# mit-acl/dpgo_ros

Measured on AMD Instinct MI355X. Metric: ms/RBCD-iteration + iterations-to-1e-6-relcost, sphere2500 5-agent, lower is better.
Workload: dtype f64; 1 GPU; sphere2500.g2o, 5 agents, synchronous round-robin RBCD, RGD(step 0.2, dense preconditioner) + Nesterov (restart 20), r=5, library weighting; mid-run iterations one launch each (k_step_fd: the private part of an agent's preconditioner product formed by the launch before its own, its row products by the one before that), hipGraphs of up to 256 iterations; agents=5, poses_per_agent=500, placement=agent a on rank a % N

## Files before the change

### dpgo_ros_amd/csrc/kernels.h

```cpp
#pragma once
#include <hip/hip_runtime.h>
#include "dpgo_dev.h"

namespace dpgo {

struct LaunchCtx {
  int r;
  hipStream_t stream;
  const AgentDev *agents;
  TeamDev *team;
  int ny = 1;
  int dense_max_n = 1 << 30;
  bool any_two_level = false;
  int tl_max_wg = 0;
  const int *host_precond = nullptr;
  const AgentDev *host_agents = nullptr;
  int num_agents = 0;
  bool bake_desc = false;
  const int *up_slots = nullptr;
  const double *up_in = nullptr;
  int up_n0 = 0, up_n1 = 0;
  int max_lds = 160 * 1024;
  int stage_cap = 0;
  const NestState *nest_all = nullptr;
// ... 29 lines not shown
void launch_eval_report(const LaunchCtx &c, int sel, int max_n, int xb, int egb, int gfb, int poff, const EvalOpts &o,
                        const ReportTail &rt);
size_t eval_staged_lds_bytes(int r, int cap);
constexpr int EVS_STATIC_LDS = 8 * 1024;
void launch_hess(const LaunchCtx &c, int sel, int max_n, int xb, int egb, int vb, int ob, int poff);
void launch_precond(const LaunchCtx &c, int sel, int max_n, int mode, int xb, int vb, int zb, int sp, int max_inner,
                    double step, int accel, int num_robots, int advance = PADV_NONE, int restart_interval = 1, int ahead = 0);
void launch_eval_stats(const LaunchCtx &c, int max_n, int first, int has_eval, int has_stats, int num_robots,
                       int restart_interval, int eval_sel = SEL_SCHED, int stats_sel = SEL_SCHED, const NestState *nest_copy = nullptr);
bool step_fe_supported(int r);
int step_fe_max_edges();
void launch_step_fe(const LaunchCtx &c, int sel, int next_sel, double step, int num_robots, int restart_interval,
                    const NestState *nest_src, NestState *nest_dst, int parity, int next2_sel = -1, int carry = 0);
int step_fe_carry_max_poses();
int step_fd_pick_m0(int min_private_chunks);
void launch_fd_open(const LaunchCtx &c, int m0, int s0, int s1, double *pacc_out);
void launch_fd_prime(const LaunchCtx &c, int s0, int s1, int s2, int max_n, int num_robots, int restart_interval, const NestState *nest_src);
void launch_step_fd(const LaunchCtx &c, int m0, int sel, int next_sel, int next2_sel, int next3_sel, double step, int num_robots,
                    int restart_interval, const NestState *nest_src, NestState *nest_dst, int parity, int flags,
                    const double *pacc_in, double *pacc_out);
constexpr int LS_MAX_TRIALS = 8;
void launch_ls_trials(const LaunchCtx &c, int sel, int max_n, int dirb, double step0, double shrink, int ntrials);
void launch_ls_cost(const LaunchCtx &c, int sel, int max_n, int dirb, int ntrials);
void launch_ls_apply(const LaunchCtx &c, int sel, int max_n, double step0, double shrink, double sigma, int ntrials, int tail = 0,
                     int num_robots = 1, int restart_interval = 1);
void launch_tcg_hv(const LaunchCtx &c, int sel, int max_n, int sp, int max_inner);
void launch_retract(const LaunchCtx &c, int sel, int max_n, int xb, int eb, double scale, int ob, int guard_state);
void launch_project_raw(const LaunchCtx &c, const double *X, double *out, int n);
void launch_tangent_raw(const LaunchCtx &c, const double *X, const double *V, double *out, int n);
void launch_retract_raw(const LaunchCtx &c, const double *X, const double *E, double *out, int n);
// ... 70 lines not shown
```

### dpgo_ros_amd/csrc/step_deep.hip

```cpp
#include "kernel_common.h"
#include <algorithm>

namespace dpgo {

constexpr int FD_KC = 2048;
#ifndef DPGO_FD_HEAD
#define DPGO_FD_HEAD 0
#endif
#ifndef DPGO_FD_GC_LATE
#define DPGO_FD_GC_LATE 0
#endif
#ifndef DPGO_FD_PACC_WT
#define DPGO_FD_PACC_WT 0
#endif
#ifndef DPGO_FD_E_EARLY
#define DPGO_FD_E_EARLY 0
#endif
#ifndef DPGO_FD_KA_PREFETCH
#define DPGO_FD_KA_PREFETCH 1
#endif
constexpr int FD_HEAD = DPGO_FD_HEAD;

enum { FD_SY_C = 0, FD_SY_E, FD_SY_D, FD_SY_F, FD_SY_N, FD_SY_RQ, FD_SY_COUNT = 8 };

__device__ __forceinline__ void fd_signal(int *cnt) {
  __builtin_amdgcn_fence(__ATOMIC_RELEASE, "workgroup", "local");
  if ((threadIdx.x & 63) == 0) __hip_atomic_fetch_add(cnt, 1, __ATOMIC_RELAXED, __HIP_MEMORY_SCOPE_WORKGROUP);
}

__device__ __forceinline__ void fd_signal_requested(int *cnt) {
  __builtin_amdgcn_sched_barrier(0);
  asm volatile("" ::: "memory");
  if ((threadIdx.x & 63) == 0) __hip_atomic_fetch_add(cnt, 1, __ATOMIC_RELAXED, __HIP_MEMORY_SCOPE_WORKGROUP);
  asm volatile("" ::: "memory");
  __builtin_amdgcn_sched_barrier(0);
}
// ... 8 lines not shown
__device__ __forceinline__ int fd_pos_off(const unsigned char *ord, int pose) {
  const int ch = pose >> 4;
  int p = 0;
#pragma unroll
  for (int i = 0; i < 32; ++i) p = ((int)ord[i] == ch) ? i : p;
  return p * 64 * R + (pose & 15) * 4 * R;
}

template <int R>
struct FdXn {
  double2 v[3][2 * R];
};

template <int R>
__device__ __forceinline__ void fd_xn_request(const AgentDev &ag, const FeBases &fb, int parity, int ln, FdXn<R> &xr) {
#pragma unroll
  for (int q = 0; q < 3; ++q) {
    {
      unsigned wsel = 0;
#pragma unroll
      for (int k = 0; k < 32; ++k) {
        const unsigned wk = ag.fe_code[(32 * q + k < FE_MAX_EDGES / 2) ? 32 * q + k : FE_MAX_EDGES / 2 - 1];
        wsel = ((ln >> 1) == k) ? wk : wsel;
      }
      const unsigned code = (ln & 1) ? (wsel >> 16) : (wsel & 0xffffu);
      const int sa = (int)(code >> 12), sf = (int)(code & 0xfffu);
      const double *yb = fb.ybase[0];
      int yn = fb.npose[0];
#pragma unroll
      for (int k = 1; k < LOOKAHEAD_MAX_AGENTS; ++k) { yb = (sa == k) ? fb.ybase[k] : yb; yn = (sa == k) ? fb.npose[k] : yn; }
      const double *xp = yb + (parity ? (size_t)B_ALT * 4 * R * yn : (size_t)0) + (size_t)sf * 4 * R;
#pragma unroll
      for (int k = 0; k < 2 * R; ++k) xr.v[q][k] = ld2(xp + 2 * k);
    }
  }
}

template <int R>
__device__ __forceinline__ void fd_xn_to_lds(const AgentDev &ag, int ln, const FdXn<R> &xr, double *Es) {
  constexpr int EPE = 4 * R + 16;
  int nsh = ag.nshared;
  asm volatile("" : "+v"(nsh));
#pragma unroll
  for (int q = 0; q < 3; ++q) {
    if (64 * q < nsh && 64 * q + ln < nsh) {
      double *E = Es + (size_t)(64 * q + ln) * EPE;
#pragma unroll
      for (int k = 0; k < 2 * R; ++k) *reinterpret_cast<double2 *>(E + 2 * k) = xr.v[q][k];
    }
  }
}

struct FdCf {
  static constexpr int TRIPS = FE_MAX_EDGES * 8 / 64;
  double2 v[TRIPS];
};

__device__ __forceinline__ void fd_cf_request(const AgentDev &ag, int ln, FdCf &cr) {
  const int nit = ag.nshared * 8;
#pragma unroll
  for (int j = 0; j < FdCf::TRIPS; ++j) cr.v[j] = ld2(ag.fe_coef + 2 * min(64 * j + ln, nit - 1));
}

template <int R>
__device__ __forceinline__ void fd_cf_to_lds(const AgentDev &ag, int ln, const FdCf &cr, double *Es) {
  constexpr int EPE = 4 * R + 16;
  int nit = ag.nshared * 8;
  asm volatile("" : "+v"(nit));
#pragma unroll
  for (int j = 0; j < FdCf::TRIPS; ++j) {
    const int t = 64 * j + ln;
    if (64 * j < nit && t < nit) *reinterpret_cast<double2 *>(Es + (size_t)(t >> 3) * EPE + 4 * R + 2 * (t & 7)) = cr.v[j];
  }
}

template <int R, int NC>
struct FdCur {
  double2 mc[NC];
  double pa[R];
};

template <int R, int M0, int NC>
__device__ __forceinline__ void fd_cur_request(const AgentDev &ag, const double *pacc_in, int bx, int nblk, int l, FdCur<R, NC> &cu) {
  const int cg = (l >> 5) & 7, kl = l & 31;
  const int N4 = ag.N4, col = 8 * bx + cg;
  const double *Mc = ag.M + (size_t)((col < N4) ? col : 0) * N4;
#pragma unroll
  for (int i = 0; i < NC; ++i) cu.mc[i] = ld2_nt(Mc + min(2 * kl + 64 * (int)ag.fe_ord[M0 + i], N4 - 2));
#pragma unroll
  for (int a = 0; a < R; ++a) cu.pa[a] = gp(pacc_in)[((size_t)min(bx, nblk - 1) * R + a) * 256 + l];
}

template <int R, int M0, int NC>
__device__ __forceinline__ void fd_cur_product(const FdCur<R, NC> &cu, const double *vs, double *red, int l) {
  const int cg = (l >> 5) & 7, kl = l & 31;
  double acc[R];
#pragma unroll
  for (int a = 0; a < R; ++a) acc[a] = cu.pa[a];
#pragma unroll
  for (int i = 0; i < NC; ++i) {
    const int k = 2 * kl + 64 * (M0 + i);
    double wv[2 * R];
#pragma unroll
    for (int q = 0; q < R; ++q) {
      const double2 t2 = *reinterpret_cast<const double2 *>(&vs[k * R + 2 * q]);
      wv[2 * q] = t2.x; wv[2 * q + 1] = t2.y;
    }
#pragma unroll
    for (int a = 0; a < R; ++a) acc[a] = __builtin_fma(wv[R + a], cu.mc[i].y, __builtin_fma(wv[a], cu.mc[i].x, acc[a]));
  }
#pragma unroll
  for (int a = 0; a < R; ++a) red[kl * (8 * R + 1) + cg * R + a] = acc[a];
}

#ifdef DPGO_FE_TRACE
#ifndef DPGO_FE_TRACE_BLOCK
#define DPGO_FE_TRACE_BLOCK 100
#endif
#define FD_TRACE_DECL __shared__ unsigned long long fd_stamps[8 * 16];
#ifndef DPGO_FD_STAMP_MASK
#define DPGO_FD_STAMP_MASK 0xFFFF
#endif
#define FD_STAMP(k) do { if (((DPGO_FD_STAMP_MASK >> (k)) & 1) && (threadIdx.x & 63) == 0) fd_stamps[(threadIdx.x >> 6) * 16 + (k)] = wall_clock64(); } while (0)
#define FD_FLUSH() do { if ((threadIdx.x & 63) == 0) { const int w_ = threadIdx.x >> 6; \
    if (blockIdx.x == DPGO_FE_TRACE_BLOCK) for (int k_ = 0; k_ < 16; ++k_) ag.part[PART_E + 4000 * PART_STRIDE + w_ * 16 + k_] = (double)fd_stamps[w_ * 16 + k_]; \
    if (w_ == 4) { ag.part[PART_E + (4100 + 2 * (int)blockIdx.x) * PART_STRIDE] = (double)fd_stamps[4 * 16]; ag.part[PART_E + (4100 + 2 * (int)blockIdx.x) * PART_STRIDE + 1] = (double)fd_stamps[4 * 16 + 15]; } \
    if (w_ == 0) { ag.part[PART_E + (4100 + 2 * (int)blockIdx.x) * PART_STRIDE + 2] = (double)fd_stamps[15]; } } } while (0)
#elif defined(DPGO_FD_ENDS)
#define FD_TRACE_DECL
#define FD_STAMP(k) do { if ((k) == 0 && blockIdx.x == 100 && threadIdx.x == 256) ag.part[PART_E + 4000 * PART_STRIDE + 64] = (double)wall_clock64(); } while (0)
#define FD_FLUSH() do { if (blockIdx.x == 100 && (threadIdx.x & 63) == 0) ag.part[PART_E + 4000 * PART_STRIDE + (threadIdx.x >> 6) * 16 + 15] = (double)wall_clock64(); } while (0)
#else
#define FD_TRACE_DECL
#define FD_STAMP(k) do { } while (0)
#define FD_FLUSH() do { } while (0)
#endif

template <int R, int M0>
__global__ __launch_bounds__(512) void k_step_fd(TeamDev *team, int sel, int next_sel, double step, int num_robots, int restart_interval,
                                                 const NestState *nest_src, NestState *nest_dst, int parity, const AgentDev agv,
                                                 int next3_sel, int flags, const FdNext nx, const FeBases fb,
                                                 const double *__restrict__ pacc_in, double *__restrict__ pacc_out, int nblk_all,
                                                 int num_agents) {
  const AgentDev &ag = agv;
#if DPGO_FD_KA_PREFETCH
  {
    const unsigned *ka = (const unsigned *)__builtin_amdgcn_kernarg_segment_ptr();
    constexpr int KA_LINES = (int)((sizeof(AgentDev) + sizeof(FdNext) + sizeof(FeBases) + 160 + 63) / 64);
    unsigned touch = 0;
#pragma unroll
    for (int i = 0; i < KA_LINES; ++i) touch |= ka[16 * i];
    asm volatile("" ::"s"(touch));
  }
#endif
  const double *__restrict__ Xr = ag.buf[parity ? B_XALT : B_X];
  const double *__restrict__ Yr = ag.buf[parity ? B_YALT : B_Y];
  double *__restrict__ Xw = ag.buf[parity ? B_X : B_XALT];
  double *__restrict__ Yw = ag.buf[parity ? B_Y : B_YALT];
  const int hb = (int)blockIdx.x;
  const int bx = (hb % 8) * ((int)gridDim.x / 8) + hb / 8;
  const int tid = threadIdx.x;
  const int N4 = ag.N4, n = ag.n;
  const int nblk = (N4 + 7) / 8;
  if (bx >= nblk_all) return;
  const bool own = bx < nblk, in = (flags & FD_IN) != 0;
  constexpr int KC = FD_KC, MREG = KC / 64, NC = MREG - M0;
  __shared__ double vs[R * KC];
  __shared__ double zs[8 * R];
  __shared__ double red[32 * (8 * R + 1)];
  __shared__ double Ysh[2 * 4 * R];
  __shared__ double Esh[2][2 * 4 * R];
  __shared__ double Es[FE_MAX_EDGES * (4 * R + 16)];
  __shared__ double tl_x[2 * 4 * R], tl_v[2 * 4 * R], tl_y[2 * 4 * R], tl_s[2 * 16];
  __shared__ double Ex[2 * 3 * 4 * R];
  __shared__ double Psh[2 * 4 * R], tl_rel[2];
  __shared__ int sy[FD_SY_COUNT];
  FD_TRACE_DECL
  FD_STAMP(0);
  if (tid < FD_SY_COUNT) sy[tid] = 0;
  lds_barrier();
  const int pj0 = own ? 2 * bx : 0, pj1 = (own && 2 * bx + 1 < n) ? 2 * bx + 1 : -1;
  const int npose = own ? ((pj1 >= 0) ? 2 : 1) : 0;
  constexpr int EPE = 4 * R + 16;
  const int cwv = __builtin_amdgcn_readfirstlane(tid >> 6), ln = tid & 63;

  if (cwv < 4) {
    const int cg = (tid >> 5) & 7, kl = tid & 31;
    for (int t = N4 * R + tid; t < KC * R; t += 256) vs[t] = 0.0;
    constexpr int NGC = ((KC - 64 * M0) * R / 2 + 255) / 256;
    double2 gc[NGC];
#if !DPGO_FD_GC_LATE
    {
      const double *Gc = ag.buf[B_CARRY_G];
#pragma unroll
      for (int u = 0; u < NGC; ++u) gc[u] = ld2(Gc + min(M0 * 64 * R + 2 * (tid + 256 * u), N4 * R - 2));
    }
#endif
    const int cold = 8 * bx + cg;
    const int N4d = nx.N4d;
    const double *Md = nx.Md + (size_t)((cold < N4d) ? cold : 0) * N4d;
    double2 mn[M0];
#pragma unroll
    for (int i = 0; i < FD_HEAD; ++i) mn[i] = ld2_nt(Md + min(2 * kl + 64 * (int)nx.ord_d[i], N4d - 2));
    FD_STAMP(10);
    __builtin_amdgcn_sched_barrier(0);
#if DPGO_FD_GC_LATE
    {
      const double *Gc = ag.buf[B_CARRY_G];
#pragma unroll
      for (int u = 0; u < NGC; ++u) gc[u] = ld2(Gc + min(M0 * 64 * R + 2 * (tid + 256 * u), N4 * R - 2));
    }
#endif
#pragma unroll
    for (int u = 0; u < NGC; ++u) {
      const int tt = M0 * 64 * R + 2 * (tid + 256 * u);
      if (tt < N4 * R) *reinterpret_cast<double2 *>(&vs[tt]) = gc[u];
    }
    fd_signal(&sy[FD_SY_C]);
    FD_STAMP(1);
    fd_wait(&sy[FD_SY_RQ], 4);
    FD_STAMP(11);
    __builtin_amdgcn_sched_barrier(0);
    asm volatile("" ::: "memory");
    constexpr int NGN = (M0 * 64 * R / 2 + 255) / 256;
    double2 gn[NGN];
#pragma unroll
    for (int u = 0; u < NGN; ++u) gn[u] = ld2(nx.Gd + min(2 * (tid + 256 * u), M0 * 64 * R - 2));
#pragma unroll
    for (int i = FD_HEAD; i < M0; ++i) mn[i] = ld2_nt(Md + min(2 * kl + 64 * (int)nx.ord_d[i], N4d - 2));
    FD_STAMP(12);
#pragma unroll
    for (int u = 0; u < NGN; ++u) {
      const int tt = 2 * (tid + 256 * u);
      if (tt < M0 * 64 * R) *reinterpret_cast<double2 *>(&vs[tt]) = gn[u];
    }
    fd_signal(&sy[FD_SY_N]);
    fd_wait(&sy[FD_SY_N], 4);
    fd_wait(&sy[FD_SY_F], 4);
    FD_STAMP(13);
    double acc[R];
#pragma unroll
    for (int a = 0; a < R; ++a) acc[a] = 0;
#pragma unroll
    for (int i = 0; i < M0; ++i) {
      const int k = 2 * kl + 64 * i;
      double wv[2 * R];
#pragma unroll
      for (int q = 0; q < R; ++q) {
        const double2 t2 = *reinterpret_cast<const double2 *>(&vs[k * R + 2 * q]);
        wv[2 * q] = t2.x; wv[2 * q + 1] = t2.y;
      }
#pragma unroll
      for (int a = 0; a < R; ++a) acc[a] = __builtin_fma(wv[R + a], mn[i].y, __builtin_fma(wv[a], mn[i].x, acc[a]));
    }
    if ((flags & FD_P) && bx < nx.nblk_d) {
#pragma unroll
#if DPGO_FD_PACC_WT
      for (int a = 0; a < R; ++a) st_c(pacc_out + ((size_t)bx * R + a) * 256 + tid, acc[a]);
#else
      for (int a = 0; a < R; ++a) gp(pacc_out)[((size_t)bx * R + a) * 256 + tid] = acc[a];
#endif
    }
    FD_STAMP(15);
    FD_FLUSH();
    return;
  }

  if (cwv < 6) {
    const int g = cwv - 4;
    const int npub = ag.npub;
    const int pq = 64 * g + ln;
    const bool pact = pq < npub;
    const int pqc = pact ? pq : 0;
    const int pj = ag.pub_pose[pqc];
    const int pe0 = ag.pub_ptr[pqc], pe1 = ag.pub_ptr[pqc + (pact ? 1 : 0)];
    double w[4 * R], x[4 * R];
    {
      const double *Wc = ag.buf[B_CARRY_W], *Xc = ag.buf[B_CARRY_X];
#pragma unroll
      for (int i = 0; i < 2 * R; ++i) {
        const double2 tw = ld2(Wc + ((size_t)i * npub + pqc) * 2), tx = ld2(Xc + ((size_t)i * npub + pqc) * 2);
        w[2 * i] = tw.x; w[2 * i + 1] = tw.y; x[2 * i] = tx.x; x[2 * i + 1] = tx.y;
      }
    }
    FD_STAMP(14);
    FdCur<R, NC> cu;
    fd_cur_request<R, M0, NC>(ag, pacc_in, bx, nblk, tid - 256, cu);
    const int npw = (nx.n_e + nblk_all - 1) / nblk_all;
    const int wls = ln / (4 * R), we = ln - wls * (4 * R);
    const int pw = bx * npw + wls;
    const bool pv = wls < 3 && wls < npw && pw < nx.n_e;
    const int pwc = pv ? pw : 0;
    const int wtile = pwc >> 6, wpl = pwc & 63, wdn = nx.soa_w_e;
    int ii[8];
#pragma unroll
    for (int u = 0; u < 8; ++u) ii[u] = gp(nx.soa_col_e)[((size_t)wtile * wdn + min(u, wdn - 1)) * 64 + wpl];
    const int qi = gp(nx.pub_index_e)[pwc];
    const int tl = tid - 256 - 64 * g;
    const size_t own_off = (size_t)((tl >= 4 * R) ? max(pj1, 0) : pj0) * 4 * R + (size_t)(tl % (4 * R));
    double pre_x = 0, pre_v = 0, pre_y = 0, pre_p = 0;
    if (tl < npose * 4 * R) {
      pre_x = gp(Xr)[own_off];
      pre_v = gp(ag.buf[B_V])[own_off];
      pre_y = gp(Yr)[own_off];
      pre_p = gp(ag.buf[B_XPREV])[own_off];
    }
    const NestState ns = nest_src[sel];
    __builtin_amdgcn_s_setprio(3);
    FD_STAMP(10);
    fd_signal_requested(&sy[FD_SY_RQ]);
    FD_STAMP(11);
    const int vs_off = fd_pos_off<R>(ag.fe_ord, pj);
    fd_wait(&sy[FD_SY_E], 2);
    FD_STAMP(1);
    if (pact) {
      double gg[4 * R];
#pragma unroll
      for (int i = 0; i < 4 * R; ++i) gg[i] = 0.0;
      for (int e = pe0; e < pe1; ++e) {
        const double *E = Es + (size_t)e * EPE;
        double xn[4 * R];
#pragma unroll
// ... 69 lines not shown
    }
    fd_wait(&sy[FD_SY_F], 4);
    if (ln < 8 * R) {
      double s = 0;
#pragma unroll
      for (int q = 0; q < 32; ++q) s += red[q * (8 * R + 1) + ln];
      zs[ln] = s;
    }
    FD_STAMP(6);
    WSYNC();
    const NestAhead nn = nest_ahead(ns, num_robots, restart_interval);
    const bool ahead_opt = next_sel == sel;
    const bool stats = in && (flags & FD_STATS) != 0, lastat = in && (flags & FD_LASTAT) != 0;
    if (ln < 2) tl_rel[ln] = 0.0;
    const TwoPoseLds tl2 = {zs, Ysh, Esh[0], Esh[1], Psh, tl_x, tl_v, tl_y, tl_s, tl_rel};
    step_two_poses<R>(ag, Xw, Yw, tl2, ln, npose, pj0, pj1, step, nn, ahead_opt, in, stats, lastat, [&](int k) { FD_STAMP(k); });
    if (stats) {
      WSYNC();
      double rl = (ln < npose) ? tl_rel[ln] : 0.0;
      rl = wave_sum(rl);
      if (ln == 0 && own) gp(ag.part)[PART_B + (size_t)bx * PART_STRIDE + 2] = rl;
    }
    FD_STAMP(15);
    FD_FLUSH();
    return;
  }

  const int h = cwv - 6;
  if (h == 0) {
    FdXn<R> er;
    fd_xn_request<R>(ag, fb, parity, ln, er);
    FD_STAMP(9);
    FdCur<R, NC> cu;
    fd_cur_request<R, M0, NC>(ag, pacc_in, bx, nblk, tid - 256, cu);
    FD_STAMP(10);
    fd_signal_requested(&sy[FD_SY_RQ]);
    FD_STAMP(11);
    __builtin_amdgcn_s_setprio(3);
    fd_xn_to_lds<R>(ag, ln, er, Es);
    fd_signal(&sy[FD_SY_E]);
    FD_STAMP(8);
    fd_wait(&sy[FD_SY_D], 2);
    fd_cur_product<R, M0, NC>(cu, vs, red, tid - 256);
    fd_signal(&sy[FD_SY_F]);
    if (bx == 0 && ln < LOOKAHEAD_MAX_AGENTS && in)
      step_books(team, nest_src, nest_dst, ln, num_agents, sel, next_sel, num_robots, restart_interval);
    FD_STAMP(14);
    FD_FLUSH();
    return;
  }

  {
    FdCf er;
    fd_cf_request(ag, ln, er);
    FD_STAMP(9);
    FdCur<R, NC> cu;
    fd_cur_request<R, M0, NC>(ag, pacc_in, bx, nblk, tid - 256, cu);
#if DPGO_FD_E_EARLY
    __builtin_amdgcn_sched_barrier(0);
    fd_cf_to_lds<R>(ag, ln, er, Es);
    fd_signal(&sy[FD_SY_E]);
    FD_STAMP(8);
    __builtin_amdgcn_sched_barrier(0);
#endif
    int pre[LOOKAHEAD_MAX_AGENTS + 1];
    pre[0] = 0;
#pragma unroll
    for (int k = 0; k < LOOKAHEAD_MAX_AGENTS; ++k) pre[k + 1] = pre[k] + ((k < num_agents) ? fb.npose[k] : 0);
    const int total = pre[LOOKAHEAD_MAX_AGENTS] - n;
    const int per = (total + nblk_all - 1) / nblk_all;
    const int q = bx * per + ln;
    const bool lact = ln < per && q < total;
    int self_lo = 0;
#pragma unroll
    for (int k = 0; k < LOOKAHEAD_MAX_AGENTS; ++k) if (k == sel) self_lo = pre[k];
// ... 6 lines not shown
    const size_t vlen = (size_t)4 * R * na_;
    double *yp = const_cast<double *>(ya);
    double *xa = yp - (size_t)(B_Y - B_X) * vlen, *va = yp + (size_t)(B_V - B_Y) * vlen;
    const size_t da = (size_t)B_ALT * vlen;
    const double *xr = parity ? xa + da : xa, *yr = parity ? yp + da : yp;
    double *oX = parity ? xa : xa + da, *oY = parity ? yp : yp + da, *oV = va;
    const int la_pose = gq - lo;
    const bool la_opt = next_sel == a;
    const size_t o = (size_t)la_pose * 4 * R;
    double la_x[4 * R], la_v[4 * R];
#pragma unroll
    for (int i = 0; i < 2 * R; ++i) {
      const double2 tx = ld2(xr + o + 2 * i), tv = ld2(va + o + 2 * i);
      la_x[2 * i] = tx.x; la_x[2 * i + 1] = tx.y; la_v[2 * i] = tv.x; la_v[2 * i + 1] = tv.y;
    }
    const NestState ns = nest_src[sel];
    FD_STAMP(10);
    fd_signal_requested(&sy[FD_SY_RQ]);
    FD_STAMP(11);
    __builtin_amdgcn_s_setprio(3);
#if !DPGO_FD_E_EARLY
    fd_cf_to_lds<R>(ag, ln, er, Es);
    fd_signal(&sy[FD_SY_E]);
    FD_STAMP(8);
#endif
    fd_wait(&sy[FD_SY_D], 2);
    fd_cur_product<R, M0, NC>(cu, vs, red, tid - 256);
    fd_signal(&sy[FD_SY_F]);
    __builtin_amdgcn_s_setprio(0);
    const NestAhead nn = nest_ahead(ns, num_robots, restart_interval);
    if (lact) {
      const bool st = in, lastat = in && (flags & FD_LASTAT) != 0;
      double *pa_ = fb.part[0];
#pragma unroll
      for (int k = 1; k < LOOKAHEAD_MAX_AGENTS; ++k) pa_ = (a == k) ? fb.part[k] : pa_;
      if (lastat) {
        double *xprev = yp - (size_t)(B_Y - B_XPREV) * vlen;
// ... 193 lines not shown
  int nblk_all = 0;
  for (int k = 0; k < c.num_agents; ++k) nblk_all = std::max(nblk_all, (c.host_agents[k].N4 + 7) / 8);
  const int gridp = ((c.host_agents[s0].N4 + 7) / 8 + 7) / 8 * 8;
  if (m0 != 24) return;
  switch (c.r) {
    case 3: hipLaunchKernelGGL((k_fd_rows<3>), dim3(nblk_all, 2), dim3(64), 0, c.stream, c.agents, s0, s1, nblk_all);
            hipLaunchKernelGGL((k_fd_partial<3, 24>), dim3(gridp), dim3(256), 0, c.stream, c.agents, s0, pacc_out); break;
    case 4: hipLaunchKernelGGL((k_fd_rows<4>), dim3(nblk_all, 2), dim3(64), 0, c.stream, c.agents, s0, s1, nblk_all);
            hipLaunchKernelGGL((k_fd_partial<4, 24>), dim3(gridp), dim3(256), 0, c.stream, c.agents, s0, pacc_out); break;
    case 5: hipLaunchKernelGGL((k_fd_rows<5>), dim3(nblk_all, 2), dim3(64), 0, c.stream, c.agents, s0, s1, nblk_all);
            hipLaunchKernelGGL((k_fd_partial<5, 24>), dim3(gridp), dim3(256), 0, c.stream, c.agents, s0, pacc_out); break;
    default: break;
  }
}

void launch_step_fd(const LaunchCtx &c, int m0, int sel, int next_sel, int next2_sel, int next3_sel, double step, int num_robots,
                    int restart_interval, const NestState *nest_src, NestState *nest_dst, int parity, int flags,
                    const double *pacc_in, double *pacc_out) {
  const AgentDev &d = c.host_agents[sel], &dd = c.host_agents[next_sel], &de = c.host_agents[next2_sel];
  int nblk_all = 0;
  for (int k = 0; k < c.num_agents; ++k) nblk_all = std::max(nblk_all, (c.host_agents[k].N4 + 7) / 8);
  const int grid = (nblk_all + 7) / 8 * 8;
  FeBases fb = {};
  for (int k = 0; k < c.num_agents && k < LOOKAHEAD_MAX_AGENTS; ++k) { fb.ybase[k] = c.host_agents[k].buf[B_Y]; fb.npose[k] = c.host_agents[k].n; fb.part[k] = c.host_agents[k].part; }
  FdNext nx = {};
  nx.Md = dd.M; nx.N4d = dd.N4; nx.nblk_d = (dd.N4 + 7) / 8; nx.Gd = dd.buf[B_CARRY_G];
  for (int i = 0; i < 32; ++i) { nx.ord_d[i] = dd.fe_ord[i]; nx.ord_e[i] = de.fe_ord[i]; }
  nx.n_e = de.n; nx.soa_w_e = de.soa_w; nx.npub_e = de.npub; nx.soa_col_e = de.soa_col; nx.soa_val_e = de.soa_val;
  nx.pub_index_e = de.pub_index; nx.Ye = de.buf[B_CARRY_Y]; nx.We = de.buf[B_CARRY_W]; nx.Xe = de.buf[B_CARRY_X]; nx.Ge = de.buf[B_CARRY_G];
#define FD_LAUNCH(RR, MM)                                                                                                   \
  hipLaunchKernelGGL((k_step_fd<RR, MM>), dim3(grid), dim3(512), 0, c.stream, c.team, sel, next_sel, step, num_robots,        \
                     restart_interval, nest_src, nest_dst, parity, d, next3_sel, flags, nx, fb, pacc_in, pacc_out, nblk_all, \
                     c.num_agents)
#define FD_LAUNCH_M(RR)                                   \
  switch (m0) {                                           \
    case 24: FD_LAUNCH(RR, 24); break;                    \
    default: break;                                       \
  }
  switch (c.r) {
    case 3: FD_LAUNCH_M(3); break;
    case 4: FD_LAUNCH_M(4); break;
    case 5: FD_LAUNCH_M(5); break;
    default: break;
  }
#undef FD_LAUNCH_M
#undef FD_LAUNCH
}

// ... 2 lines not shown
```

### dpgo_ros_amd/csrc/team_run.hip

```cpp
#include "team_internal.h"

using namespace dpgo;
using namespace dpgo_host;

namespace dpgo_host {

void drop_graphs(dpgo_team *t) {
  for (auto &kv : t->graphs) if (kv.second) (void)hipGraphExecDestroy(kv.second);
  t->graphs.clear();
  t->graph_flip.clear();
}

int check_exchange_error(dpgo_team *t) {
  if (!t->h_bar_err || !*t->h_bar_err) return 0;
  const int code = *t->h_bar_err;
  *t->h_bar_err = 0;
  drop_graphs(t);
  set_err("an in-kernel exchange timed out (code " + std::to_string(code) + ": 2 hand-off of the one-launch RTR solve, 3 two-level "
          "preconditioner, 4 mailbox of the device-side UPDATE token): the iterates since the last successful synchronisation are invalid");
  return DPGO_ERR;
}

static void revalidate_graphs(dpgo_team *t) { if (!t->graph_valid) { drop_graphs(t); t->graph_valid = true; } }

// ... 64 lines not shown
  for (int q = 0; q < P; ++q)
    for (int u = 1; u < 4; ++u)
      if (t->sched[(size_t)q] == t->sched[(size_t)((q + u) % P)]) return 0;
  int min_priv = 32, nblk_all = 0, total = 0;
  for (auto &a : t->ag) {
    if (a->npub < 1 || a->npub > 128 || !a->dev.fe_code_ok || (int)a->se_host.size() > FE_MAX_EDGES) return 0;
    min_priv = std::min(min_priv, a->dev.fe_npriv);
    nblk_all = std::max(nblk_all, (4 * a->n + 7) / 8);
    total += a->n;
  }
  for (auto &a : t->ag)
    if ((total - a->n + nblk_all - 1) / nblk_all > 64) return 0;
  int m0 = step_fd_pick_m0(min_priv);
  if (const char *e = std::getenv("DPGO_FD_M0")) { const int f = std::atoi(e); if (f > 0 && f <= min_priv && step_fd_pick_m0(f) == f) m0 = f; }
  if (m0 == 0) return 0;
  const size_t want = (size_t)2 * nblk_all * t->prm.r * 256;
  if (t->d_fd_pacc.n < want && t->d_fd_pacc.alloc(want)) return 0;
  return m0;
}

struct RunPlan {
  bool graphable;
  bool ls;
  bool pipelined;
  bool bake;
  bool fe_ok;
  int fd_m0, P;
};

static RunPlan make_plan(dpgo_team *t) {
// ... 369 lines not shown
```

Baseline: 13.01 us.

## Pack hot kernel arguments into a compact head and defer bulk kernarg reads

Restructures k_step_fd's argument list so that the values needed first (buffer base, M, pacc_in, fe_coef, and packed n/npub/nshared/parity/flags/order ids) sit in a small leading header of scalar kernargs. The large AgentDev/FdNext/FeBases block moves behind it and is read only after the first global loads are issued. The goal is to shorten the kernel's startup latency by not stalling on many scalar kernarg loads before issuing memory requests. It also swaps the 32-way select for the edge code with a binary tree and moves some own-pose loads earlier. The fd path is now gated on a host check that the agent's buffers sit in one allocation and fit the packed field widths, so agents that fail the check fall back to the slower path.

```diff
diff --git a/dpgo_ros_amd/csrc/kernels.h b/dpgo_ros_amd/csrc/kernels.h
--- a/dpgo_ros_amd/csrc/kernels.h
+++ b/dpgo_ros_amd/csrc/kernels.h
@@ -67,6 +67,7 @@
                     const NestState *nest_src, NestState *nest_dst, int parity, int next2_sel = -1, int carry = 0);
 int step_fe_carry_max_poses();
 int step_fd_pick_m0(int min_private_chunks);
+bool step_fd_head_ok(const AgentDev &d, int r, int m0);
 void launch_fd_open(const LaunchCtx &c, int m0, int s0, int s1, double *pacc_out);
 void launch_fd_prime(const LaunchCtx &c, int s0, int s1, int s2, int max_n, int num_robots, int restart_interval, const NestState *nest_src);
 void launch_step_fd(const LaunchCtx &c, int m0, int sel, int next_sel, int next2_sel, int next3_sel, double step, int num_robots,
diff --git a/dpgo_ros_amd/csrc/step_deep.hip b/dpgo_ros_amd/csrc/step_deep.hip
--- a/dpgo_ros_amd/csrc/step_deep.hip
+++ b/dpgo_ros_amd/csrc/step_deep.hip
@@ -1,12 +1,10 @@
 #include "kernel_common.h"
+#include "step_head.h"
 #include <algorithm>
 
 namespace dpgo {
 
 constexpr int FD_KC = 2048;
-#ifndef DPGO_FD_HEAD
-#define DPGO_FD_HEAD 0
-#endif
 #ifndef DPGO_FD_GC_LATE
 #define DPGO_FD_GC_LATE 0
 #endif
@@ -19,7 +17,6 @@
 #ifndef DPGO_FD_KA_PREFETCH
 #define DPGO_FD_KA_PREFETCH 1
 #endif
-constexpr int FD_HEAD = DPGO_FD_HEAD;
 
 enum { FD_SY_C = 0, FD_SY_E, FD_SY_D, FD_SY_F, FD_SY_N, FD_SY_RQ, FD_SY_COUNT = 8 };
 
@@ -58,21 +55,32 @@
 
 template <int R>
 __device__ __forceinline__ void fd_xn_request(const AgentDev &ag, const FeBases &fb, int parity, int ln, FdXn<R> &xr) {
+  const double *ybs[LOOKAHEAD_MAX_AGENTS];
+  int yns[LOOKAHEAD_MAX_AGENTS];
+#pragma unroll
+  for (int k = 0; k < LOOKAHEAD_MAX_AGENTS; ++k) { ybs[k] = fb.ybase[k]; yns[k] = fb.npose[k]; }
+  static_assert(LOOKAHEAD_MAX_AGENTS == 8, "one operand below per agent");
+  asm volatile("" : "+s"(ybs[0]), "+s"(ybs[1]), "+s"(ybs[2]), "+s"(ybs[3]), "+s"(ybs[4]), "+s"(ybs[5]), "+s"(ybs[6]), "+s"(ybs[7]),
+               "+s"(yns[0]), "+s"(yns[1]), "+s"(yns[2]), "+s"(yns[3]), "+s"(yns[4]), "+s"(yns[5]), "+s"(yns[6]), "+s"(yns[7]));
 #pragma unroll
   for (int q = 0; q < 3; ++q) {
     {
-      unsigned wsel = 0;
-#pragma unroll
-      for (int k = 0; k < 32; ++k) {
-        const unsigned wk = ag.fe_code[(32 * q + k < FE_MAX_EDGES / 2) ? 32 * q + k : FE_MAX_EDGES / 2 - 1];
-        wsel = ((ln >> 1) == k) ? wk : wsel;
-      }
+      unsigned wt[32];
+#pragma unroll
+      for (int k = 0; k < 32; ++k) wt[k] = ag.fe_code[(32 * q + k < FE_MAX_EDGES / 2) ? 32 * q + k : FE_MAX_EDGES / 2 - 1];
+#pragma unroll
+      for (int bit = 0; bit < 5; ++bit) {
+        const bool up = ((ln >> 1) >> bit) & 1;
+#pragma unroll
+        for (int k = 0; k < (16 >> bit); ++k) wt[k] = up ? wt[2 * k + 1] : wt[2 * k];
+      }
+      const unsigned wsel = wt[0];
       const unsigned code = (ln & 1) ? (wsel >> 16) : (wsel & 0xffffu);
       const int sa = (int)(code >> 12), sf = (int)(code & 0xfffu);
-      const double *yb = fb.ybase[0];
-      int yn = fb.npose[0];
-#pragma unroll
-      for (int k = 1; k < LOOKAHEAD_MAX_AGENTS; ++k) { yb = (sa == k) ? fb.ybase[k] : yb; yn = (sa == k) ? fb.npose[k] : yn; }
+      const double *yb = ybs[0];
+      int yn = yns[0];
+#pragma unroll
+      for (int k = 1; k < LOOKAHEAD_MAX_AGENTS; ++k) { yb = (sa == k) ? ybs[k] : yb; yn = (sa == k) ? yns[k] : yn; }
       const double *xp = yb + (parity ? (size_t)B_ALT * 4 * R * yn : (size_t)0) + (size_t)sf * 4 * R;
 #pragma unroll
       for (int k = 0; k < 2 * R; ++k) xr.v[q][k] = ld2(xp + 2 * k);
@@ -81,9 +89,9 @@
 }
 
 template <int R>
-__device__ __forceinline__ void fd_xn_to_lds(const AgentDev &ag, int ln, const FdXn<R> &xr, double *Es) {
+__device__ __forceinline__ void fd_xn_to_lds(int nshared, int ln, const FdXn<R> &xr, double *Es) {
   constexpr int EPE = 4 * R + 16;
-  int nsh = ag.nshared;
+  int nsh = nshared;
   asm volatile("" : "+v"(nsh));
 #pragma unroll
   for (int q = 0; q < 3; ++q) {
@@ -100,16 +108,16 @@
   double2 v[TRIPS];
 };
 
-__device__ __forceinline__ void fd_cf_request(const AgentDev &ag, int ln, FdCf &cr) {
-  const int nit = ag.nshared * 8;
-#pragma unroll
-  for (int j = 0; j < FdCf::TRIPS; ++j) cr.v[j] = ld2(ag.fe_coef + 2 * min(64 * j + ln, nit - 1));
+__device__ __forceinline__ void fd_cf_request(const double *fe_coef, int nshared, int ln, FdCf &cr) {
+  const int nit = nshared * 8;
+#pragma unroll
+  for (int j = 0; j < FdCf::TRIPS; ++j) cr.v[j] = ld2(fe_coef + 2 * min(64 * j + ln, nit - 1));
 }
 
 template <int R>
-__device__ __forceinline__ void fd_cf_to_lds(const AgentDev &ag, int ln, const FdCf &cr, double *Es) {
+__device__ __forceinline__ void fd_cf_to_lds(int nshared, int ln, const FdCf &cr, double *Es) {
   constexpr int EPE = 4 * R + 16;
-  int nit = ag.nshared * 8;
+  int nit = nshared * 8;
   asm volatile("" : "+v"(nit));
 #pragma unroll
   for (int j = 0; j < FdCf::TRIPS; ++j) {
@@ -125,12 +133,14 @@
 };
 
 template <int R, int M0, int NC>
-__device__ __forceinline__ void fd_cur_request(const AgentDev &ag, const double *pacc_in, int bx, int nblk, int l, FdCur<R, NC> &cu) {
+__device__ __forceinline__ void fd_cur_request(const FdHead &hd, int N4, int bx, int nblk, int l, FdCur<R, NC> &cu) {
+  static_assert(NC <= FD_HEAD_ORD_MAX && M0 + NC == 32, "the head holds the ids of the last chunks");
   const int cg = (l >> 5) & 7, kl = l & 31;
-  const int N4 = ag.N4, col = 8 * bx + cg;
-  const double *Mc = ag.M + (size_t)((col < N4) ? col : 0) * N4;
-#pragma unroll
-  for (int i = 0; i < NC; ++i) cu.mc[i] = ld2_nt(Mc + min(2 * kl + 64 * (int)ag.fe_ord[M0 + i], N4 - 2));
+  const int col = 8 * bx + cg;
+  const double *pacc_in = hd.pacc_in;
+  const double *Mc = hd.M + (size_t)((col < N4) ? col : 0) * N4;
+#pragma unroll
+  for (int i = 0; i < NC; ++i) cu.mc[i] = ld2_nt(Mc + min(2 * kl + 64 * fd_head_ord(hd.ord_lo, hd.ord_hi, i), N4 - 2));
 #pragma unroll
   for (int a = 0; a < R; ++a) cu.pa[a] = gp(pacc_in)[((size_t)min(bx, nblk - 1) * R + a) * 256 + l];
 }
@@ -157,6 +167,7 @@
   for (int a = 0; a < R; ++a) red[kl * (8 * R + 1) + cg * R + a] = acc[a];
 }
 
+#define FD_TRACE_PART (fd_args_behind_requests<false>().ag.part)
 #ifdef DPGO_FE_TRACE
 #ifndef DPGO_FE_TRACE_BLOCK
 #define DPGO_FE_TRACE_BLOCK 100
@@ -167,44 +178,65 @@
 #endif
 #define FD_STAMP(k) do { if (((DPGO_FD_STAMP_MASK >> (k)) & 1) && (threadIdx.x & 63) == 0) fd_stamps[(threadIdx.x >> 6) * 16 + (k)] = wall_clock64(); } while (0)
 #define FD_FLUSH() do { if ((threadIdx.x & 63) == 0) { const int w_ = threadIdx.x >> 6; \
-    if (blockIdx.x == DPGO_FE_TRACE_BLOCK) for (int k_ = 0; k_ < 16; ++k_) ag.part[PART_E + 4000 * PART_STRIDE + w_ * 16 + k_] = (double)fd_stamps[w_ * 16 + k_]; \
-    if (w_ == 4) { ag.part[PART_E + (4100 + 2 * (int)blockIdx.x) * PART_STRIDE] = (double)fd_stamps[4 * 16]; ag.part[PART_E + (4100 + 2 * (int)blockIdx.x) * PART_STRIDE + 1] = (double)fd_stamps[4 * 16 + 15]; } \
-    if (w_ == 0) { ag.part[PART_E + (4100 + 2 * (int)blockIdx.x) * PART_STRIDE + 2] = (double)fd_stamps[15]; } } } while (0)
+    if (blockIdx.x == DPGO_FE_TRACE_BLOCK) for (int k_ = 0; k_ < 16; ++k_) FD_TRACE_PART[PART_E + 4000 * PART_STRIDE + w_ * 16 + k_] = (double)fd_stamps[w_ * 16 + k_]; \
+    if (w_ == 4) { FD_TRACE_PART[PART_E + (4100 + 2 * (int)blockIdx.x) * PART_STRIDE] = (double)fd_stamps[4 * 16]; FD_TRACE_PART[PART_E + (4100 + 2 * (int)blockIdx.x) * PART_STRIDE + 1] = (double)fd_stamps[4 * 16 + 15]; } \
+    if (w_ == 0) { FD_TRACE_PART[PART_E + (4100 + 2 * (int)blockIdx.x) * PART_STRIDE + 2] = (double)fd_stamps[15]; } } } while (0)
 #elif defined(DPGO_FD_ENDS)
 #define FD_TRACE_DECL
-#define FD_STAMP(k) do { if ((k) == 0 && blockIdx.x == 100 && threadIdx.x == 256) ag.part[PART_E + 4000 * PART_STRIDE + 64] = (double)wall_clock64(); } while (0)
-#define FD_FLUSH() do { if (blockIdx.x == 100 && (threadIdx.x & 63) == 0) ag.part[PART_E + 4000 * PART_STRIDE + (threadIdx.x >> 6) * 16 + 15] = (double)wall_clock64(); } while (0)
+#define FD_STAMP(k) do { if ((k) == 0 && blockIdx.x == 100 && threadIdx.x == 256) FD_TRACE_PART[PART_E + 4000 * PART_STRIDE + 64] = (double)wall_clock64(); } while (0)
+#define FD_FLUSH() do { if (blockIdx.x == 100 && (threadIdx.x & 63) == 0) FD_TRACE_PART[PART_E + 4000 * PART_STRIDE + (threadIdx.x >> 6) * 16 + 15] = (double)wall_clock64(); } while (0)
 #else
 #define FD_TRACE_DECL
 #define FD_STAMP(k) do { } while (0)
 #define FD_FLUSH() do { } while (0)
 #endif
 
+struct FdArgs {
+  AgentDev ag;
+  FdNext nx;
+  FeBases fb;
+  TeamDev *team;
+  const NestState *nest_src;
+  NestState *nest_dst;
+  double *pacc_out;
+  double step;
+  int sel, next_sel, next3_sel, num_robots, restart_interval, num_agents;
+};
+
+constexpr size_t FD_ARGS_OFFSET = (4 * FD_HEAD_DWORDS + alignof(FdArgs) - 1) / alignof(FdArgs) * alignof(FdArgs);
+template <bool TOUCH>
+__device__ __forceinline__ const FdArgs &fd_args_behind_requests() {
+  typedef const __attribute__((address_space(4))) char *SegPtr;
+  __builtin_amdgcn_sched_barrier(0);
+  SegPtr p = (SegPtr)__builtin_amdgcn_kernarg_segment_ptr() + FD_ARGS_OFFSET;
+  asm volatile("" : "+s"(p)::"memory");
+#if DPGO_FD_KA_PREFETCH
+  if constexpr (TOUCH) {
+    const __attribute__((address_space(4))) unsigned *ka = (const __attribute__((address_space(4))) unsigned *)p;
+    static_assert(sizeof(FdArgs) > 19 * 64 && sizeof(FdArgs) <= 20 * 64, "one operand below for every line of FdArgs");
+    constexpr int LAST = (int)(sizeof(FdArgs) / 4) - 1;
+    asm volatile("" ::"s"(ka[0]), "s"(ka[16]), "s"(ka[32]), "s"(ka[48]), "s"(ka[64]), "s"(ka[80]), "s"(ka[96]), "s"(ka[112]),
+                 "s"(ka[128]), "s"(ka[144]), "s"(ka[160]), "s"(ka[176]), "s"(ka[192]), "s"(ka[208]), "s"(ka[224]), "s"(ka[240]),
+                 "s"(ka[256]), "s"(ka[272]), "s"(ka[288]), "s"(ka[304]), "s"(ka[LAST]));
+  }
+#endif
+  return *(const FdArgs *)p;
+}
+
 template <int R, int M0>
-__global__ __launch_bounds__(512) void k_step_fd(TeamDev *team, int sel, int next_sel, double step, int num_robots, int restart_interval,
-                                                 const NestState *nest_src, NestState *nest_dst, int parity, const AgentDev agv,
-                                                 int next3_sel, int flags, const FdNext nx, const FeBases fb,
-                                                 const double *__restrict__ pacc_in, double *__restrict__ pacc_out, int nblk_all,
-                                                 int num_agents) {
-  const AgentDev &ag = agv;
-#if DPGO_FD_KA_PREFETCH
-  {
-    const unsigned *ka = (const unsigned *)__builtin_amdgcn_kernarg_segment_ptr();
-    constexpr int KA_LINES = (int)((sizeof(AgentDev) + sizeof(FdNext) + sizeof(FeBases) + 160 + 63) / 64);
-    unsigned touch = 0;
-#pragma unroll
-    for (int i = 0; i < KA_LINES; ++i) touch |= ka[16 * i];
-    asm volatile("" ::"s"(touch));
-  }
-#endif
-  const double *__restrict__ Xr = ag.buf[parity ? B_XALT : B_X];
-  const double *__restrict__ Yr = ag.buf[parity ? B_YALT : B_Y];
-  double *__restrict__ Xw = ag.buf[parity ? B_X : B_XALT];
-  double *__restrict__ Yw = ag.buf[parity ? B_Y : B_YALT];
+__global__ __launch_bounds__(512) void k_step_fd(double *hd_buf0, const double *hd_M, const double *__restrict__ hd_pacc_in,
+                                                 const double *hd_fe_coef, unsigned hd_np, unsigned hd_sf, unsigned hd_ord_lo,
+                                                 unsigned hd_ord_hi, int nblk_all, const FdArgs fa) {
+  const FdHead hd = {hd_buf0, hd_M, hd_pacc_in, hd_fe_coef, hd_np, hd_sf, hd_ord_lo, hd_ord_hi, nblk_all};
+  const int n = fd_head_n(hd.np), N4 = 4 * n, hd_npub = fd_head_npub(hd.np), hd_nshared = fd_head_nshared(hd.sf);
+  const int parity = fd_head_parity(hd.sf), flags = fd_head_flags(hd.sf);
+  const double *__restrict__ Xr = fd_head_buf(hd.buf0, R, n, parity ? B_XALT : B_X);
+  const double *__restrict__ Yr = fd_head_buf(hd.buf0, R, n, parity ? B_YALT : B_Y);
+  double *__restrict__ Xw = fd_head_buf(hd.buf0, R, n, parity ? B_X : B_XALT);
+  double *__restrict__ Yw = fd_head_buf(hd.buf0, R, n, parity ? B_Y : B_YALT);
   const int hb = (int)blockIdx.x;
-  const int bx = (hb % 8) * ((int)gridDim.x / 8) + hb / 8;
+  const int bx = (hb % 8) * ((nblk_all + 7) / 8) + hb / 8;
   const int tid = threadIdx.x;
-  const int N4 = ag.N4, n = ag.n;
   const int nblk = (N4 + 7) / 8;
   if (bx >= nblk_all) return;
   const bool own = bx < nblk, in = (flags & FD_IN) != 0;
@@ -233,24 +265,23 @@
     for (int t = N4 * R + tid; t < KC * R; t += 256) vs[t] = 0.0;
     constexpr int NGC = ((KC - 64 * M0) * R / 2 + 255) / 256;
     double2 gc[NGC];
+    const double *Gc = fd_head_buf(hd.buf0, R, n, B_CARRY_G);
 #if !DPGO_FD_GC_LATE
     {
-      const double *Gc = ag.buf[B_CARRY_G];
 #pragma unroll
       for (int u = 0; u < NGC; ++u) gc[u] = ld2(Gc + min(M0 * 64 * R + 2 * (tid + 256 * u), N4 * R - 2));
     }
 #endif
+    const FdArgs &as = fd_args_behind_requests<false>();
+    const FdNext &nx = as.nx;
     const int cold = 8 * bx + cg;
     const int N4d = nx.N4d;
     const double *Md = nx.Md + (size_t)((cold < N4d) ? cold : 0) * N4d;
     double2 mn[M0];
-#pragma unroll
-    for (int i = 0; i < FD_HEAD; ++i) mn[i] = ld2_nt(Md + min(2 * kl + 64 * (int)nx.ord_d[i], N4d - 2));
     FD_STAMP(10);
     __builtin_amdgcn_sched_barrier(0);
 #if DPGO_FD_GC_LATE
     {
-      const double *Gc = ag.buf[B_CARRY_G];
 #pragma unroll
       for (int u = 0; u < NGC; ++u) gc[u] = ld2(Gc + min(M0 * 64 * R + 2 * (tid + 256 * u), N4 * R - 2));
     }
@@ -271,7 +302,7 @@
 #pragma unroll
     for (int u = 0; u < NGN; ++u) gn[u] = ld2(nx.Gd + min(2 * (tid + 256 * u), M0 * 64 * R - 2));
 #pragma unroll
-    for (int i = FD_HEAD; i < M0; ++i) mn[i] = ld2_nt(Md + min(2 * kl + 64 * (int)nx.ord_d[i], N4d - 2));
+    for (int i = 0; i < M0; ++i) mn[i] = ld2_nt(Md + min(2 * kl + 64 * (int)nx.ord_d[i], N4d - 2));
     FD_STAMP(12);
 #pragma unroll
     for (int u = 0; u < NGN; ++u) {
@@ -287,6 +318,10 @@
     for (int a = 0; a < R; ++a) acc[a] = 0;
 #pragma unroll
     for (int i = 0; i < M0; ++i) {
+      if (i % 8 == 0 && i > 0) {
+#pragma unroll
+        for (int a = 0; a < R; ++a) asm volatile("" : "+v"(acc[a])::"memory");
+      }
       const int k = 2 * kl + 64 * i;
       double wv[2 * R];
 #pragma unroll
@@ -300,9 +335,9 @@
     if ((flags & FD_P) && bx < nx.nblk_d) {
 #pragma unroll
 #if DPGO_FD_PACC_WT
-      for (int a = 0; a < R; ++a) st_c(pacc_out + ((size_t)bx * R + a) * 256 + tid, acc[a]);
+      for (int a = 0; a < R; ++a) st_c(as.pacc_out + ((size_t)bx * R + a) * 256 + tid, acc[a]);
 #else
-      for (int a = 0; a < R; ++a) gp(pacc_out)[((size_t)bx * R + a) * 256 + tid] = acc[a];
+      for (int a = 0; a < R; ++a) gp(as.pacc_out)[((size_t)bx * R + a) * 256 + tid] = acc[a];
 #endif
     }
     FD_STAMP(15);
@@ -312,15 +347,13 @@
 
   if (cwv < 6) {
     const int g = cwv - 4;
-    const int npub = ag.npub;
+    const int npub = hd_npub;
     const int pq = 64 * g + ln;
     const bool pact = pq < npub;
     const int pqc = pact ? pq : 0;
-    const int pj = ag.pub_pose[pqc];
-    const int pe0 = ag.pub_ptr[pqc], pe1 = ag.pub_ptr[pqc + (pact ? 1 : 0)];
     double w[4 * R], x[4 * R];
     {
-      const double *Wc = ag.buf[B_CARRY_W], *Xc = ag.buf[B_CARRY_X];
+      const double *Wc = fd_head_buf(hd.buf0, R, n, B_CARRY_W), *Xc = fd_head_buf(hd.buf0, R, n, B_CARRY_X);
 #pragma unroll
       for (int i = 0; i < 2 * R; ++i) {
         const double2 tw = ld2(Wc + ((size_t)i * npub + pqc) * 2), tx = ld2(Xc + ((size_t)i * npub + pqc) * 2);
@@ -329,7 +362,21 @@
     }
     FD_STAMP(14);
     FdCur<R, NC> cu;
-    fd_cur_request<R, M0, NC>(ag, pacc_in, bx, nblk, tid - 256, cu);
+    fd_cur_request<R, M0, NC>(hd, N4, bx, nblk, tid - 256, cu);
+    const int tl = tid - 256 - 64 * g;
+    const size_t own_off = (size_t)((tl >= 4 * R) ? max(pj1, 0) : pj0) * 4 * R + (size_t)(tl % (4 * R));
+    double pre_x = 0, pre_v = 0, pre_y = 0, pre_p = 0;
+    if (tl < npose * 4 * R) {
+      pre_x = gp(Xr)[own_off];
+      pre_v = gp(fd_head_buf(hd.buf0, R, n, B_V))[own_off];
+      pre_y = gp(Yr)[own_off];
+      pre_p = gp(fd_head_buf(hd.buf0, R, n, B_XPREV))[own_off];
+    }
+    const FdArgs &as = fd_args_behind_requests<true>();
+    const AgentDev &ag = as.ag;
+    const FdNext &nx = as.nx;
+    const int pj = ag.pub_pose[pqc];
+    const int pe0 = ag.pub_ptr[pqc], pe1 = ag.pub_ptr[pqc + (pact ? 1 : 0)];
     const int npw = (nx.n_e + nblk_all - 1) / nblk_all;
     const int wls = ln / (4 * R), we = ln - wls * (4 * R);
     const int pw = bx * npw + wls;
@@ -340,16 +387,8 @@
 #pragma unroll
     for (int u = 0; u < 8; ++u) ii[u] = gp(nx.soa_col_e)[((size_t)wtile * wdn + min(u, wdn - 1)) * 64 + wpl];
     const int qi = gp(nx.pub_index_e)[pwc];
-    const int tl = tid - 256 - 64 * g;
-    const size_t own_off = (size_t)((tl >= 4 * R) ? max(pj1, 0) : pj0) * 4 * R + (size_t)(tl % (4 * R));
-    double pre_x = 0, pre_v = 0, pre_y = 0, pre_p = 0;
-    if (tl < npose * 4 * R) {
-      pre_x = gp(Xr)[own_off];
-      pre_v = gp(ag.buf[B_V])[own_off];
-      pre_y = gp(Yr)[own_off];
-      pre_p = gp(ag.buf[B_XPREV])[own_off];
-    }
-    const NestState ns = nest_src[sel];
+    const int sel = as.sel, next_sel = as.next_sel, num_robots = as.num_robots, restart_interval = as.restart_interval;
+    const NestState ns = as.nest_src[sel];
     __builtin_amdgcn_s_setprio(3);
     FD_STAMP(10);
     fd_signal_requested(&sy[FD_SY_RQ]);
@@ -449,7 +488,7 @@
     const bool stats = in && (flags & FD_STATS) != 0, lastat = in && (flags & FD_LASTAT) != 0;
     if (ln < 2) tl_rel[ln] = 0.0;
     const TwoPoseLds tl2 = {zs, Ysh, Esh[0], Esh[1], Psh, tl_x, tl_v, tl_y, tl_s, tl_rel};
-    step_two_poses<R>(ag, Xw, Yw, tl2, ln, npose, pj0, pj1, step, nn, ahead_opt, in, stats, lastat, [&](int k) { FD_STAMP(k); });
+    step_two_poses<R>(ag, Xw, Yw, tl2, ln, npose, pj0, pj1, as.step, nn, ahead_opt, in, stats, lastat, [&](int k) { FD_STAMP(k); });
     if (stats) {
       WSYNC();
       double rl = (ln < npose) ? tl_rel[ln] : 0.0;
@@ -463,23 +502,24 @@
 
   const int h = cwv - 6;
   if (h == 0) {
+    FdCur<R, NC> cu;
+    fd_cur_request<R, M0, NC>(hd, N4, bx, nblk, tid - 256, cu);
+    const FdArgs &as = fd_args_behind_requests<true>();
     FdXn<R> er;
-    fd_xn_request<R>(ag, fb, parity, ln, er);
+    fd_xn_request<R>(as.ag, as.fb, parity, ln, er);
     FD_STAMP(9);
-    FdCur<R, NC> cu;
-    fd_cur_request<R, M0, NC>(ag, pacc_in, bx, nblk, tid - 256, cu);
     FD_STAMP(10);
     fd_signal_requested(&sy[FD_SY_RQ]);
     FD_STAMP(11);
     __builtin_amdgcn_s_setprio(3);
-    fd_xn_to_lds<R>(ag, ln, er, Es);
+    fd_xn_to_lds<R>(hd_nshared, ln, er, Es);
     fd_signal(&sy[FD_SY_E]);
     FD_STAMP(8);
     fd_wait(&sy[FD_SY_D], 2);
     fd_cur_product<R, M0, NC>(cu, vs, red, tid - 256);
     fd_signal(&sy[FD_SY_F]);
     if (bx == 0 && ln < LOOKAHEAD_MAX_AGENTS && in)
-      step_books(team, nest_src, nest_dst, ln, num_agents, sel, next_sel, num_robots, restart_interval);
+      step_books(as.team, as.nest_src, as.nest_dst, ln, as.num_agents, as.sel, as.next_sel, as.num_robots, as.restart_interval);
     FD_STAMP(14);
     FD_FLUSH();
     return;
@@ -487,13 +527,17 @@
 
   {
     FdCf er;
-    fd_cf_request(ag, ln, er);
+    fd_cf_request(hd.fe_coef, hd_nshared, ln, er);
     FD_STAMP(9);
     FdCur<R, NC> cu;
-    fd_cur_request<R, M0, NC>(ag, pacc_in, bx, nblk, tid - 256, cu);
+    fd_cur_request<R, M0, NC>(hd, N4, bx, nblk, tid - 256, cu);
+    const FdArgs &as = fd_args_behind_requests<true>();
+    const FeBases &fb = as.fb;
+    const int sel = as.sel, next_sel = as.next_sel, next3_sel = as.next3_sel, num_agents = as.num_agents;
+    const int num_robots = as.num_robots, restart_interval = as.restart_interval;
 #if DPGO_FD_E_EARLY
     __builtin_amdgcn_sched_barrier(0);
-    fd_cf_to_lds<R>(ag, ln, er, Es);
+    fd_cf_to_lds<R>(hd_nshared, ln, er, Es);
     fd_signal(&sy[FD_SY_E]);
     FD_STAMP(8);
     __builtin_amdgcn_sched_barrier(0);
@@ -530,13 +574,13 @@
       const double2 tx = ld2(xr + o + 2 * i), tv = ld2(va + o + 2 * i);
       la_x[2 * i] = tx.x; la_x[2 * i + 1] = tx.y; la_v[2 * i] = tv.x; la_v[2 * i + 1] = tv.y;
     }
-    const NestState ns = nest_src[sel];
+    const NestState ns = as.nest_src[sel];
     FD_STAMP(10);
     fd_signal_requested(&sy[FD_SY_RQ]);
     FD_STAMP(11);
     __builtin_amdgcn_s_setprio(3);
 #if !DPGO_FD_E_EARLY
-    fd_cf_to_lds<R>(ag, ln, er, Es);
+    fd_cf_to_lds<R>(hd_nshared, ln, er, Es);
     fd_signal(&sy[FD_SY_E]);
     FD_STAMP(8);
 #endif
@@ -760,6 +804,12 @@
   }
 }
 
+bool step_fd_head_ok(const AgentDev &d, int r, int m0) {
+  FdHead hd;
+  return fd_head_build(hd, d.buf, NBUF, r, d.n, d.N4, d.npub, d.nshared, d.M, d.fe_coef, d.fe_ord, m0, 1, FD_HEAD_FLAGS_MAX, nullptr,
+                       (d.N4 + 7) / 8);
+}
+
 void launch_step_fd(const LaunchCtx &c, int m0, int sel, int next_sel, int next2_sel, int next3_sel, double step, int num_robots,
                     int restart_interval, const NestState *nest_src, NestState *nest_dst, int parity, int flags,
                     const double *pacc_in, double *pacc_out) {
@@ -767,17 +817,24 @@
   int nblk_all = 0;
   for (int k = 0; k < c.num_agents; ++k) nblk_all = std::max(nblk_all, (c.host_agents[k].N4 + 7) / 8);
   const int grid = (nblk_all + 7) / 8 * 8;
-  FeBases fb = {};
+  FdArgs fa = {};
+  FeBases &fb = fa.fb;
+  FdNext &nx = fa.nx;
   for (int k = 0; k < c.num_agents && k < LOOKAHEAD_MAX_AGENTS; ++k) { fb.ybase[k] = c.host_agents[k].buf[B_Y]; fb.npose[k] = c.host_agents[k].n; fb.part[k] = c.host_agents[k].part; }
-  FdNext nx = {};
   nx.Md = dd.M; nx.N4d = dd.N4; nx.nblk_d = (dd.N4 + 7) / 8; nx.Gd = dd.buf[B_CARRY_G];
   for (int i = 0; i < 32; ++i) { nx.ord_d[i] = dd.fe_ord[i]; nx.ord_e[i] = de.fe_ord[i]; }
   nx.n_e = de.n; nx.soa_w_e = de.soa_w; nx.npub_e = de.npub; nx.soa_col_e = de.soa_col; nx.soa_val_e = de.soa_val;
   nx.pub_index_e = de.pub_index; nx.Ye = de.buf[B_CARRY_Y]; nx.We = de.buf[B_CARRY_W]; nx.Xe = de.buf[B_CARRY_X]; nx.Ge = de.buf[B_CARRY_G];
-#define FD_LAUNCH(RR, MM)                                                                                                   \
-  hipLaunchKernelGGL((k_step_fd<RR, MM>), dim3(grid), dim3(512), 0, c.stream, c.team, sel, next_sel, step, num_robots,        \
-                     restart_interval, nest_src, nest_dst, parity, d, next3_sel, flags, nx, fb, pacc_in, pacc_out, nblk_all, \
-                     c.num_agents)
+  fa.ag = d;
+  fa.team = c.team; fa.nest_src = nest_src; fa.nest_dst = nest_dst; fa.pacc_out = pacc_out; fa.step = step;
+  fa.sel = sel; fa.next_sel = next_sel; fa.next3_sel = next3_sel; fa.num_robots = num_robots;
+  fa.restart_interval = restart_interval; fa.num_agents = c.num_agents;
+  FdHead hd;
+  if (!fd_head_build(hd, d.buf, NBUF, c.r, d.n, d.N4, d.npub, d.nshared, d.M, d.fe_coef, d.fe_ord, m0, parity, flags, pacc_in, nblk_all))
+    return;
+#define FD_LAUNCH(RR, MM)                                                                                                    \
+  hipLaunchKernelGGL((k_step_fd<RR, MM>), dim3(grid), dim3(512), 0, c.stream, hd.buf0, hd.M, hd.pacc_in, hd.fe_coef, hd.np, \
+                     hd.sf, hd.ord_lo, hd.ord_hi, hd.nblk_all, fa)
 #define FD_LAUNCH_M(RR)                                   \
   switch (m0) {                                           \
     case 24: FD_LAUNCH(RR, 24); break;                    \
diff --git a/dpgo_ros_amd/csrc/step_head.h b/dpgo_ros_amd/csrc/step_head.h
--- /dev/null
+++ b/dpgo_ros_amd/csrc/step_head.h
@@ -0,0 +1,67 @@
+#pragma once
+#include <cstddef>
+
+#ifndef DPGO_HD
+#if defined(__HIPCC__)
+#define DPGO_HD __host__ __device__ __forceinline__
+#else
+#define DPGO_HD inline
+#endif
+#endif
+
+namespace dpgo {
+
+constexpr int FD_HEAD_DWORDS = 13;
+constexpr int FD_HEAD_N_MAX = 512, FD_HEAD_NPUB_MAX = 128, FD_HEAD_NSHARED_MAX = 160, FD_HEAD_FLAGS_MAX = 63;
+constexpr int FD_HEAD_ORD_MAX = 8;
+
+struct FdHead {
+  double *buf0;
+  const double *M, *pacc_in, *fe_coef;
+  unsigned np, sf, ord_lo, ord_hi;
+  int nblk_all;
+};
+
+DPGO_HD unsigned fd_head_pack_np(int n, int npub) { return (unsigned)n | ((unsigned)npub << 16); }
+DPGO_HD int fd_head_n(unsigned np) { return (int)(np & 0xffffu); }
+DPGO_HD int fd_head_npub(unsigned np) { return (int)(np >> 16); }
+
+DPGO_HD unsigned fd_head_pack_sf(int nshared, int parity, int flags) { return (unsigned)nshared | ((unsigned)parity << 8) | ((unsigned)flags << 9); }
+DPGO_HD int fd_head_nshared(unsigned sf) { return (int)(sf & 0xffu); }
+DPGO_HD int fd_head_parity(unsigned sf) { return (int)((sf >> 8) & 1u); }
+DPGO_HD int fd_head_flags(unsigned sf) { return (int)(sf >> 9); }
+
+DPGO_HD int fd_head_ord(unsigned ord_lo, unsigned ord_hi, int i) { return (int)(((i < 4 ? ord_lo : ord_hi) >> (8 * (i & 3))) & 0xffu); }
+
+DPGO_HD double *fd_head_buf(double *buf0, int r, int n, int b) { return buf0 + (size_t)4 * r * n * b; }
+
+DPGO_HD bool fd_head_fits(int n, int N4, int npub, int nshared, int parity, int flags, int m0) {
+  return n >= 1 && n <= FD_HEAD_N_MAX && N4 == 4 * n && npub >= 0 && npub <= FD_HEAD_NPUB_MAX && nshared >= 0 &&
+         nshared <= FD_HEAD_NSHARED_MAX && (parity == 0 || parity == 1) && flags >= 0 && flags <= FD_HEAD_FLAGS_MAX &&
+         m0 >= 32 - FD_HEAD_ORD_MAX && m0 <= 32;
+}
+
+DPGO_HD bool fd_head_one_allocation(double *const *buf, int nbuf, int r, int n) {
+  for (int b = 0; b < nbuf; ++b)
+    if (buf[b] != fd_head_buf(buf[0], r, n, b)) return false;
+  return true;
+}
+
+DPGO_HD bool fd_head_build(FdHead &h, double *const *buf, int nbuf, int r, int n, int N4, int npub, int nshared, const double *M,
+                           const double *fe_coef, const unsigned char *ord, int m0, int parity, int flags,
+                           const double *pacc_in, int nblk_all) {
+  if (!fd_head_fits(n, N4, npub, nshared, parity, flags, m0) || nblk_all < (N4 + 7) / 8 || !fd_head_one_allocation(buf, nbuf, r, n))
+    return false;
+  h.buf0 = buf[0]; h.M = M; h.pacc_in = pacc_in; h.fe_coef = fe_coef;
+  h.np = fd_head_pack_np(n, npub);
+  h.sf = fd_head_pack_sf(nshared, parity, flags);
+  h.ord_lo = h.ord_hi = 0;
+  for (int i = 0; m0 + i < 32; ++i) {
+    const unsigned v = (unsigned)ord[m0 + i] << (8 * (i & 3));
+    if (i < 4) h.ord_lo |= v; else h.ord_hi |= v;
+  }
+  h.nblk_all = nblk_all;
+  return true;
+}
+
+}
diff --git a/dpgo_ros_amd/csrc/team_run.hip b/dpgo_ros_amd/csrc/team_run.hip
--- a/dpgo_ros_amd/csrc/team_run.hip
+++ b/dpgo_ros_amd/csrc/team_run.hip
@@ -102,6 +102,8 @@
   int m0 = step_fd_pick_m0(min_priv);
   if (const char *e = std::getenv("DPGO_FD_M0")) { const int f = std::atoi(e); if (f > 0 && f <= min_priv && step_fd_pick_m0(f) == f) m0 = f; }
   if (m0 == 0) return 0;
+  for (auto &a : t->ag)
+    if (!step_fd_head_ok(a->dev, t->prm.r, m0)) return 0;
   const size_t want = (size_t)2 * nblk_all * t->prm.r * 256;
   if (t->d_fd_pacc.n < want && t->d_fd_pacc.alloc(want)) return 0;
   return m0;
```

Result: faster. 12.00 us, median of 6 (-7.7%).
